# Cognoscan/entropy_coders

Measured on AMD Instinct MI355X. Metric: FSE encode+decode GiB/s on 1 GiB synthetic bytes; bit-exact round-trip, higher is better.
Workload: dtype u8

## Files before the change

entropy_coders_amd/csrc/fse_capi.cpp:

```cpp
#include <hip/hip_runtime.h>
#include <stdio.h>
#include <stdlib.h>
#include <string.h>

#include <algorithm>
#include <atomic>
#include <memory>
#include <mutex>
#include <thread>
#include <vector>

#include "../../include/fsehip.h"
#include "fse_kernels.h"

namespace {

constexpr uint32_t kDefaultBlock = 65536;
constexpr uint32_t kMaxBlock = 1u << 28;

uint64_t round_up(uint64_t x, uint64_t a) { return (x + a - 1) / a * a; }

enum {
    SCRATCH_DT = 0,
    SCRATCH_DTINFO = 1,
// ... 222 lines not shown
    uint8_t* buf[2] = {};
    size_t cap[2] = {};
    ~PinnedStaging() { release(); }
    void release() {
        for (int i = 0; i < 2; ++i) {
            if (buf[i]) (void)hipHostFree(buf[i]);
            buf[i] = nullptr;
            cap[i] = 0;
        }
    }
    uint8_t* get(int i, size_t bytes) {
        if (cap[i] < bytes) {
            if (buf[i]) (void)hipHostFree(buf[i]);
            buf[i] = nullptr;
            cap[i] = 0;
            void* p = nullptr;
            const size_t want = round_up(std::max<size_t>(bytes, size_t(64) << 10), 4096);
            if (hipHostMalloc(&p, want, hipHostMallocDefault) != hipSuccess) return nullptr;
            buf[i] = static_cast<uint8_t*>(p);
            cap[i] = want;
        }
        return buf[i];
    }
};
thread_local PinnedStaging g_pin;

struct Meta {
    uint32_t comp_len;
    uint32_t payload_bits;
    int32_t status;
    uint32_t pad;
};

int compress_one(const uint8_t* src, size_t n, uint32_t table_log, uint8_t* dst, size_t dst_cap, size_t* dst_len,
                 uint64_t* payload_bits, uint32_t nstates = 2) {
    if (!dst_len) return FSE_ERR_BAD_ARG;
    if (n == 0) return FSE_ERR_EMPTY;
    if (n > kMaxBlock) return FSE_ERR_UNSUPPORTED;
    if (table_log > 15) table_log = 15;
    if (!device_ok()) return FSE_ERR_NO_DEVICE;
    fsehip_params p{(uint32_t)round_up(n, 16), table_log, 0, table_log ? std::max<uint32_t>(table_log, 11) : 11,
                    nstates};
    const uint64_t slot = fsehip_slot_bytes(p.block_size, p.max_table_log);
    const size_t in_bytes = round_up(n, 16);
    const size_t pin_out = std::min<size_t>(slot, kPinOut);
    uint8_t* d_src = g_stage.get(0, in_bytes + 16);
    uint8_t* d_out = g_stage.get(1, slot);
    uint8_t* d_meta = g_stage.get(2, sizeof(Meta));
    uint8_t* h_in = g_pin.get(0, in_bytes);
    uint8_t* h_ret = g_pin.get(1, 256 + pin_out);
    if (!d_src || !d_out || !d_meta || !h_in || !h_ret) return FSE_ERR_HIP;
    memcpy(h_in, src, n);
    auto fail = [](int rc) {
        (void)hipStreamSynchronize(nullptr);
        return rc;
    };
    if (hipMemcpyAsync(d_src, h_in, in_bytes, hipMemcpyHostToDevice, nullptr) != hipSuccess) return fail(FSE_ERR_HIP);
    Meta* m = reinterpret_cast<Meta*>(d_meta);
    int rc = fsehip_compress_blocks(&p, d_src, n, d_out, slot, &m->comp_len, &m->payload_bits, nullptr,
                                    &m->status, nullptr);
    if (rc) return fail(rc);
    if (fsehip::launch_host_return(d_meta, d_out, &m->comp_len, h_ret, h_ret + 256, (uint32_t)pin_out, nullptr) !=
        hipSuccess)
        return fail(FSE_ERR_HIP);
    if (hipStreamSynchronize(nullptr) != hipSuccess) return FSE_ERR_HIP;
    Meta h;
    memcpy(&h, h_ret, sizeof h);
    if (h.status != FSE_OK) return h.status;
    if (*dst_len > dst_cap || dst_cap - *dst_len < h.comp_len) return FSE_ERR_DST_TOO_SMALL;
    const size_t head = std::min<size_t>(h.comp_len, pin_out);
    memcpy(dst + *dst_len, h_ret + 256, head);
    if (h.comp_len > head &&
        hipMemcpy(dst + *dst_len + head, d_out + head, h.comp_len - head, hipMemcpyDeviceToHost) != hipSuccess)
        return FSE_ERR_HIP;
    *dst_len += h.comp_len;
    if (payload_bits) *payload_bits = h.payload_bits;
    return FSE_OK;
}

}

extern "C" {

uint64_t fsehip_slot_bytes(uint32_t block_size, uint32_t max_table_log) {
    const uint64_t L = max_table_log ? max_table_log : 12;
    const uint64_t payload = ((uint64_t)block_size * L + 2 * L + 1 + 7) / 8;
    return round_up(512 + payload + 16, 256);
}

uint32_t fsehip_sidecar_per_block(uint32_t block_size, uint32_t ckpt_interval) {
    if (ckpt_interval == 0) return 0;
    return block_size / 2u / ckpt_interval + 2u;
}

uint32_t fsehip_sidecar_per_block_ns(uint32_t block_size, uint32_t ckpt_interval, uint32_t nstates) {
    if (ckpt_interval == 0) return 0;
    return nstates == 1 ? block_size / ckpt_interval + 2u : block_size / 2u / ckpt_interval + 2u;
}

int fsehip_device_count(void) {
    int n = 0;
    if (hipGetDeviceCount(&n) != hipSuccess) return 0;
    return n;
}

#ifdef FSEHIP_DIAG
const char* fsehip_version(void) { return "fsehip 0.2 (gfx950, diagnostics build: environment knobs live)"; }
#else
const char* fsehip_version(void) { return "fsehip 0.2 (gfx950)"; }
#endif

int fsehip_release_workspace(int device, fsehip_stream_t stream) {
    const int rc = release_workspaces(device, stream, false);
    g_stage.release();
    g_pin.release();
    return rc;
}

static int compress_blocks_impl(const fsehip_params* p, const uint8_t* d_src, uint64_t n_total, uint8_t* d_out,
                                uint64_t slot_bytes, uint32_t* d_comp_len, uint32_t* d_payload_bits,
                                uint64_t* d_sidecar, int32_t* d_status, fsehip_stream_t stream, Lease* held) {
    if (!p || !d_src || !d_out || !d_comp_len || !d_status) return FSE_ERR_BAD_ARG;
    if (n_total == 0) return FSE_ERR_EMPTY;
    const uint32_t bs = p->block_size ? p->block_size : kDefaultBlock;
    if (bs > kMaxBlock) return FSE_ERR_UNSUPPORTED;
    const uint64_t n_blocks = (n_total + bs - 1) / bs;
    if (n_blocks > 1 && (bs & 15u)) return FSE_ERR_BAD_ARG;
    if (n_blocks > 0xFFFFFFFFull) return FSE_ERR_BAD_ARG;
    const uint32_t lmax = kern_lmax(lmax_for(p));
    if (slot_bytes & 15u) return FSE_ERR_BAD_ARG;
    const uint32_t ns = p->nstates == 1 ? 1u : 2u;
    if (p->nstates > 2) return FSE_ERR_BAD_ARG;
    if (p->ckpt_interval && (p->ckpt_interval < (ns == 1 ? 16u : 8u) || (p->ckpt_interval & (p->ckpt_interval - 1))))
        return FSE_ERR_BAD_ARG;
    if (!device_ok()) return FSE_ERR_NO_DEVICE;
    fsehip::EncParams P{};
    P.nstates = ns;
    P.src = d_src;
    P.n_total = n_total;
    P.block_size = bs;
    P.n_blocks = (uint32_t)n_blocks;
    P.table_log = p->table_log;
    P.ckpt_interval = d_sidecar ? p->ckpt_interval : 0;
    P.ckpt_per_block = fsehip_sidecar_per_block_ns(bs, P.ckpt_interval, ns);
    P.out = d_out;
    P.slot_bytes = slot_bytes;
    P.comp_len = d_comp_len;
    P.payload_bits = d_payload_bits;
    P.sidecar = P.ckpt_interval ? d_sidecar : nullptr;
    P.status = d_status;
    P.lanes = (ns == 2 && env_u32("FSEHIP_ENC_LANES", 64) == 32) ? 32 : 64;
    P.debug = env_u32("FSEHIP_DEBUG", 0);
    P.xlds = env_u32("FSEHIP_ENC_XLDS", 0);
    P.rank_inject = env_u32("FSEHIP_RANK_INJECT", 0);
    const size_t groups = (n_blocks * P.lanes + 63) / 64;
    P.stamps = g_stamps_enc.get(groups);
    std::unique_ptr<Lease> lease;
    if (fsehip::enc_gsym(lmax) && slot_bytes < fsehip::ENC_SPREAD_OFF + (1ull << lmax)) {
        if (!held) lease = std::make_unique<Lease>(stream);
        P.spread = static_cast<uint8_t*>((held ? held : lease.get())->get(SCRATCH_SPREAD, n_blocks << lmax));
        if (!P.spread) return FSE_ERR_HIP;
    }
    hipError_t e = fsehip::launch_encode(P, lmax, static_cast<hipStream_t>(stream));
    if (P.stamps) g_stamps_enc.report("encode", groups, static_cast<hipStream_t>(stream));
    return e == hipSuccess ? FSE_OK : FSE_ERR_HIP;
}

int fsehip_compress_blocks(const fsehip_params* p, const uint8_t* d_src, uint64_t n_total, uint8_t* d_out,
                           uint64_t slot_bytes, uint32_t* d_comp_len, uint32_t* d_payload_bits, uint64_t* d_sidecar,
                           int32_t* d_status, fsehip_stream_t stream) {
    return compress_blocks_impl(p, d_src, n_total, d_out, slot_bytes, d_comp_len, d_payload_bits, d_sidecar, d_status,
                                stream, nullptr);
}

uint64_t fsehip_stream_out_bytes(uint32_t src_len, uint32_t max_table_log) {
    const uint64_t L = max_table_log ? std::min<uint32_t>(max_table_log, 15u) : 12;
    return round_up(512 + ((uint64_t)src_len * L + 2 * L + 1 + 7) / 8, 16);
}

int fsehip_compress_streams(uint32_t nstates, uint32_t table_log, uint32_t max_table_log, const uint8_t* d_src,
                            const fsehip_stream_desc* d_desc, uint32_t n_streams, uint8_t* d_out,
                            uint32_t* d_comp_len, uint32_t* d_payload_bits, int32_t* d_status,
                            fsehip_stream_t stream) {
    if (n_streams == 0) return FSE_OK;
    if (nstates > 2 || !d_src || !d_desc || !d_out || !d_comp_len || !d_status ||
        (reinterpret_cast<uintptr_t>(d_src) & 15u) || (reinterpret_cast<uintptr_t>(d_out) & 15u))
        return FSE_ERR_BAD_ARG;
    if (n_streams > (1u << 24) || max_table_log > 15) return FSE_ERR_UNSUPPORTED;
    if (!device_ok()) return FSE_ERR_NO_DEVICE;
    if (table_log > 15) table_log = 15;
    if (table_log && table_log < 5) table_log = 5;
    const fsehip_params p{0, table_log, 0, max_table_log, nstates};
    const uint32_t lmax = kern_lmax(lmax_for(&p));
    fsehip::EncParams P{};
    P.nstates = nstates == 1 ? 1u : 2u;
    P.src = d_src;
    P.n_blocks = n_streams;
    P.table_log = table_log;
    P.out = d_out;
    P.comp_len = d_comp_len;
    P.payload_bits = d_payload_bits;
    P.status = d_status;
    P.lanes = 64;
    P.desc = d_desc;
    std::unique_ptr<Lease> lease;
    if (fsehip::enc_gsym(lmax)) {
        lease = std::make_unique<Lease>(stream);
        P.spread = static_cast<uint8_t*>(lease->get(SCRATCH_SPREAD, (uint64_t)n_streams << lmax));
        if (!P.spread) return FSE_ERR_HIP;
    }
    return fsehip::launch_encode(P, lmax, static_cast<hipStream_t>(stream)) == hipSuccess ? FSE_OK : FSE_ERR_HIP;
}

static void defer_symbols(Lease& lease, fsehip::DecParams& P, uint32_t lmax) {
    if (lmax > 11 || P.block_size < 2u || P.n_blocks >= (1u << 24) || !env_u32("FSEHIP_SERIAL_DEFER", 1)) return;
    P.bulk = static_cast<uint32_t*>(lease.get(SCRATCH_BULK, 8ull * P.n_blocks, true));
    P.states = P.bulk ? static_cast<uint32_t*>(lease.get(SCRATCH_STATES, 2ull * P.n_blocks * P.block_size, true))
                      : nullptr;
    if (!P.states || !P.bulk) P.states = P.bulk = nullptr;
}

static int decompress_impl(const fsehip_params* p, const uint8_t* d_in, uint64_t slot_bytes,
                           const uint32_t* d_comp_len, const uint64_t* d_sidecar, uint8_t* d_out, uint64_t n_total,
                           uint64_t* d_sidecar_out, int32_t* d_status, uint32_t* d_out_len, uint32_t out_cap,
                           fsehip_stream_t stream, const uint32_t* d_dt, const int32_t* d_dtinfo,
                           Lease* lease = nullptr) {
    if (!p || !d_in || !d_comp_len || !d_out || !d_status || !d_dt || !d_dtinfo) return FSE_ERR_BAD_ARG;
    const uint32_t bs = p->block_size ? p->block_size : kDefaultBlock;
    if (bs > kMaxBlock) return FSE_ERR_UNSUPPORTED;
    const uint64_t n_blocks = n_total ? (n_total + bs - 1) / bs : 1;
    if (n_blocks > 1 && (bs & 15u)) return FSE_ERR_BAD_ARG;
    if (n_blocks > 0xFFFFFFFFull) return FSE_ERR_BAD_ARG;
    if ((slot_bytes & 31u) || (reinterpret_cast<uintptr_t>(d_in) & 15u) || (reinterpret_cast<uintptr_t>(d_out) & 15u))
        return FSE_ERR_BAD_ARG;
    const uint32_t ns = p->nstates == 1 ? 1u : 2u;
    if (p->nstates > 2) return FSE_ERR_BAD_ARG;
    if ((d_sidecar || d_sidecar_out) &&
        (p->ckpt_interval < (ns == 1 ? 16u : 8u) || (p->ckpt_interval & (p->ckpt_interval - 1))))
        return FSE_ERR_BAD_ARG;
    if (ns == 1 && d_sidecar_out && kern_lmax(p->max_table_log) > 12) return FSE_ERR_UNSUPPORTED;
    if (!device_ok()) return FSE_ERR_NO_DEVICE;
    fsehip::DecParams P{};
    P.nstates = ns;
    P.in = d_in;
    P.slot_bytes = slot_bytes;
    P.comp_len = d_comp_len;
    P.sidecar = d_sidecar;
    P.ckpt_interval = p->ckpt_interval;
    P.ckpt_per_block = fsehip_sidecar_per_block_ns(bs, p->ckpt_interval, ns);
    P.out = d_out;
    P.n_total = n_total;
    P.block_size = bs;
    P.n_blocks = (uint32_t)n_blocks;
    P.out_cap = out_cap;
    P.status = d_status;
    P.out_len = d_out_len;
    P.sidecar_out = d_sidecar_out;
    P.dt = d_dt;
    P.dtinfo = d_dtinfo;
    if (lease && !d_sidecar && !d_sidecar_out) defer_symbols(*lease, P, kern_lmax(p->max_table_log));
    P.stamps = g_stamps_dec.get(n_blocks);
    hipError_t e = fsehip::launch_decode(P, kern_lmax(p->max_table_log), static_cast<hipStream_t>(stream));
    if (P.stamps) g_stamps_dec.report("decode", n_blocks, static_cast<hipStream_t>(stream));
    return e == hipSuccess ? FSE_OK : FSE_ERR_HIP;
}

uint64_t fsehip_dtable_bytes(uint32_t max_table_log) { return 4ull << kern_lmax(max_table_log); }

static int build_dtables_impl(const fsehip_params* p, const uint8_t* d_in, uint64_t slot_bytes,
                              const uint32_t* d_comp_len, uint32_t n_blocks, uint32_t* d_dtables, int32_t* d_dtinfo,
                              fsehip_stream_t stream, Lease* lease) {
    if (!p || !d_in || !d_comp_len || !d_dtables || !d_dtinfo || (slot_bytes & 255u)) return FSE_ERR_BAD_ARG;
    if (n_blocks == 0) return FSE_OK;
    if (!device_ok()) return FSE_ERR_NO_DEVICE;
    fsehip::DtParams D{};
    if (lease && n_blocks >= 256u && kern_lmax(p->max_table_log) <= 12 && !env_u32("FSEHIP_DT_WAVE_PARSE", 0)) {
        uint8_t* h = static_cast<uint8_t*>(lease->get(SCRATCH_HDR, fsehip::hdr_scratch_bytes(n_blocks), true));
        if (h) {
            D.hdr_norm = reinterpret_cast<uint32_t*>(h);
            D.hdr_meta = reinterpret_cast<int2*>(h + 512ull * n_blocks);
        }
    }
    D.in = d_in;
    D.slot_bytes = slot_bytes;
    D.comp_len = d_comp_len;
    D.n_blocks = n_blocks;
    D.dt = d_dtables;
    D.dtinfo = d_dtinfo;
    D.xlds = env_u32("FSEHIP_DT_XLDS", 0);
    D.rank_inject = env_u32("FSEHIP_RANK_INJECT", 0);
    D.stamps = g_stamps_dt.get(n_blocks);
    hipError_t e = fsehip::launch_dtables(D, kern_lmax(p->max_table_log), static_cast<hipStream_t>(stream));
    if (D.stamps) g_stamps_dt.report("dtables", n_blocks, static_cast<hipStream_t>(stream));
    return e == hipSuccess ? FSE_OK : FSE_ERR_HIP;
}

int fsehip_build_dtables(const fsehip_params* p, const uint8_t* d_in, uint64_t slot_bytes, const uint32_t* d_comp_len,
                         uint32_t n_blocks, uint32_t* d_dtables, int32_t* d_dtinfo, fsehip_stream_t stream) {
    if (n_blocks < 256u) return build_dtables_impl(p, d_in, slot_bytes, d_comp_len, n_blocks, d_dtables, d_dtinfo, stream,
                                                   nullptr);
    Lease lease(stream);
    return build_dtables_impl(p, d_in, slot_bytes, d_comp_len, n_blocks, d_dtables, d_dtinfo, stream, &lease);
}

int fsehip_decompress_blocks_dt(const fsehip_params* p, const uint8_t* d_in, uint64_t slot_bytes,
                                const uint32_t* d_comp_len, const uint64_t* d_sidecar, const uint32_t* d_dtables,
                                const int32_t* d_dtinfo, uint8_t* d_out, uint64_t n_total, int32_t* d_status,
                                fsehip_stream_t stream) {
    if (n_total == 0) return FSE_ERR_EMPTY;
    if (!p || !d_dtables || !d_dtinfo) return FSE_ERR_BAD_ARG;
    if (d_sidecar && p->ckpt_interval == 0) return FSE_ERR_BAD_ARG;
    if (d_sidecar)
        return decompress_impl(p, d_in, slot_bytes, d_comp_len, d_sidecar, d_out, n_total, nullptr, d_status, nullptr,
                               0, stream, d_dtables, d_dtinfo);
    Lease lease(stream);
    return decompress_impl(p, d_in, slot_bytes, d_comp_len, nullptr, d_out, n_total, nullptr, d_status, nullptr, 0,
                           stream, d_dtables, d_dtinfo, &lease);
}

extern "C++" {
template <class Run>
static int with_dtables_lease(const fsehip_params* p, const uint8_t* d_in, uint64_t slot_bytes,
                              const uint32_t* d_comp_len, uint64_t n_blocks, fsehip_stream_t stream, Lease& lease,
                              Run run) {
    uint32_t* dt = static_cast<uint32_t*>(lease.get(SCRATCH_DT, fsehip_dtable_bytes(p->max_table_log) * n_blocks));
    int32_t* info = static_cast<int32_t*>(lease.get(SCRATCH_DTINFO, 4ull * n_blocks));
    if (!dt || !info) return FSE_ERR_HIP;
    int rc = build_dtables_impl(p, d_in, slot_bytes, d_comp_len, (uint32_t)n_blocks, dt, info, stream, &lease);
    return rc != FSE_OK ? rc : run(dt, info, lease);
}
template <class Run>
static int with_dtables_n(const fsehip_params* p, const uint8_t* d_in, uint64_t slot_bytes, const uint32_t* d_comp_len,
                          uint64_t n_blocks, fsehip_stream_t stream, Run run) {
    if (n_blocks > 0xFFFFFFFFull) return FSE_ERR_BAD_ARG;
    if (!device_ok()) return FSE_ERR_NO_DEVICE;
    Lease lease(stream);
    return with_dtables_lease(p, d_in, slot_bytes, d_comp_len, n_blocks, stream, lease, run);
}
template <class Run>
static int with_dtables(const fsehip_params* p, const uint8_t* d_in, uint64_t slot_bytes, const uint32_t* d_comp_len,
                        uint64_t n_total, fsehip_stream_t stream, Run run) {
    const uint32_t bs = p->block_size ? p->block_size : kDefaultBlock;
    if (bs > kMaxBlock) return FSE_ERR_UNSUPPORTED;
    return with_dtables_n(p, d_in, slot_bytes, d_comp_len, (n_total + bs - 1) / bs, stream, run);
}
}

int fsehip_decompress_blocks(const fsehip_params* p, const uint8_t* d_in, uint64_t slot_bytes,
                             const uint32_t* d_comp_len, const uint64_t* d_sidecar, uint8_t* d_out, uint64_t n_total,
                             int32_t* d_status, fsehip_stream_t stream) {
    if (n_total == 0) return FSE_ERR_EMPTY;
    if (!p) return FSE_ERR_BAD_ARG;
    if (d_sidecar && p->ckpt_interval == 0) return FSE_ERR_BAD_ARG;
    return with_dtables(p, d_in, slot_bytes, d_comp_len, n_total, stream,
                        [&](const uint32_t* dt, const int32_t* info, Lease& lease) {
                            return decompress_impl(p, d_in, slot_bytes, d_comp_len, d_sidecar, d_out, n_total, nullptr,
// ... 1043 lines not shown
```

entropy_coders_amd/csrc/fse_kernels.h:

```cpp
#pragma once
#include <hip/hip_runtime.h>
#include <stdint.h>

#include "../../include/fsehip.h"

namespace fsehip {

struct EncParams {
    const uint8_t* src;
    uint64_t n_total;
    uint32_t block_size;
    uint32_t n_blocks;
    uint32_t table_log;
    uint32_t ckpt_interval;
    uint32_t ckpt_per_block;
    uint8_t* out;
    uint64_t slot_bytes;
    uint32_t* comp_len;
    uint32_t* payload_bits;
    uint64_t* sidecar;
    int32_t* status;
    uint32_t lanes;
    uint32_t nstates;
    uint32_t debug;
    uint64_t* stamps;
    uint32_t xlds;
    uint32_t peer_ranks;
    uint32_t rank_inject;
    uint8_t* spread;
    const fsehip_stream_desc* desc;
};
constexpr bool enc_gsym(uint32_t lmax) { return lmax >= 13u; }
constexpr uint32_t ENC_SPREAD_OFF = 512;

struct DecParams {
    const uint8_t* in;
    uint64_t slot_bytes;
    const uint32_t* comp_len;
    const uint64_t* sidecar;
    uint32_t ckpt_interval;
    uint32_t ckpt_per_block;
    uint8_t* out;
    uint64_t n_total;
    uint32_t block_size;
    uint32_t n_blocks;
    uint32_t out_cap;
    int32_t* status;
    uint32_t* out_len;
    uint64_t* sidecar_out;
    uint64_t* stamps;
    const uint32_t* dt;
    const int32_t* dtinfo;
    uint32_t pass;
    uint32_t nstates;
    uint32_t* states;
    uint32_t* bulk;
};

struct DtParams {
    const uint8_t* in;
    uint64_t slot_bytes;
    const uint32_t* comp_len;
    uint32_t n_blocks;
    uint32_t* dt;
    int32_t* dtinfo;
    uint32_t xlds;
    uint64_t* stamps;
    int2* hdr_meta;
    uint32_t* hdr_norm;
    uint32_t peer_ranks;
    uint32_t rank_inject;
};
constexpr uint64_t hdr_scratch_bytes(uint64_t n_blocks) { return n_blocks * (512u + 8u); }

struct GenParams {
    uint8_t* out;
    uint64_t n_total;
    uint64_t block_size;
    uint64_t seed;
    int32_t kind;
    uint32_t nsym;
    uint16_t bound[1024];
};

struct NormArgs {
    int mode;
    const uint8_t* src;
    uint64_t n;
    const uint32_t* counts;
    uint32_t size, table_len, log2;
    fse_norm_histogram* out;
    uint32_t* counts_out;
    int32_t* status;
};
hipError_t launch_norm(const NormArgs& A, hipStream_t s);
hipError_t launch_hdr_write(const fse_norm_histogram* nh, uint8_t* out, uint32_t* bits, int32_t* status, hipStream_t s);
hipError_t launch_hdr_read(const uint8_t* src, uint32_t n, fse_norm_histogram* out, uint32_t* used, int32_t* status,
                           hipStream_t s);
hipError_t launch_table(const fse_norm_histogram* nh, int enc, fse_encode_table* et, fse_decode_table* dt,
                        int32_t* status, hipStream_t s);
hipError_t rank_order_check(uint32_t* violations, uint64_t* atomics);
hipError_t rank_fallbacks_enc(uint32_t* out, bool reset);
hipError_t rank_fallbacks_dec(uint32_t* out, bool reset);
hipError_t rank_fallbacks_tab(uint32_t* out, bool reset);
bool atomic_ranks_on();
int rank_mode(int mode);
hipError_t launch_host_return(const void* meta, const uint8_t* src, const uint32_t* len, void* hmeta, uint8_t* hdst,
                              uint32_t max, hipStream_t s);
uint64_t bits_tiles(uint64_t count);
hipError_t launch_bits_scan(const uint8_t* nbits, const uint8_t* ops, uint64_t count, uint32_t* tile_sum,
                            uint64_t* tile_off, uint64_t* total, hipStream_t s);
hipError_t launch_bits_pack(const uint32_t* vals, const uint8_t* nbits, uint64_t count, const uint64_t* tile_off,
                            const uint64_t* total, uint32_t* out, uint64_t lim_words, hipStream_t s);
hipError_t launch_bits_unpack(const uint8_t* in, uint64_t n_bytes, uint64_t total_bits, int stack,
                              const uint8_t* nbits, const uint8_t* ops, uint64_t count, const uint64_t* tile_off,
                              const uint64_t* total, uint32_t* vals, uint64_t* result, hipStream_t s);

#ifndef FSEHIP_KSTAMPS
#define FSEHIP_KSTAMPS
constexpr int kStamps = 10;
#endif
constexpr int32_t FSE_DEFERRED = 1;

hipError_t launch_encode(const EncParams& P, uint32_t lmax, hipStream_t stream);
hipError_t launch_dtables(const DtParams& P, uint32_t lmax, hipStream_t stream);
hipError_t launch_decode(const DecParams& P, uint32_t lmax, hipStream_t stream);
hipError_t launch_single(const DecParams& P, uint32_t lmax, hipStream_t stream);
constexpr uint32_t single_ftab_bytes() { return 2048u * 8u; }
int occupancy_report(char* buf, int cap);
int occupancy_report_dec(char* buf, int cap);
hipError_t launch_histogram(const uint8_t* src, uint64_t n_total, uint32_t block_size, uint32_t n_blocks,
                            uint32_t* counts, uint32_t* table_len, hipStream_t stream);
hipError_t launch_generate(const GenParams& G, hipStream_t stream);
hipError_t launch_pack(const uint8_t* slots, uint64_t slot_bytes, const uint32_t* comp_len, const uint64_t* offsets,
                       uint32_t n_blocks, uint8_t* stream, int unpack, hipStream_t hs);
hipError_t launch_copy(const uint8_t* src, const uint64_t* src_off, const uint32_t* lens, uint32_t n_blocks,
                       uint8_t* dst, const uint64_t* dst_off, hipStream_t hs);

hipError_t launch_stream_offsets(const uint32_t* lens, uint32_t n, uint64_t* offsets, uint64_t* total,
                                 hipStream_t hs);

struct FrameHdr {
    uint32_t w[8];
};
struct FrameChunk {
    uint8_t* frame;
    uint64_t frame_len;
    uint64_t n_total;
    uint32_t block_size, ckpt_interval, nstates, n_blocks;
    uint32_t c0, cb;
    uint8_t* slots;
    uint64_t slot_bytes;
    uint32_t* comp_len;
    int32_t* status;
    uint64_t* sidecar;
    uint32_t spb;
    uint32_t* kind;
    uint64_t* off;
    uint64_t* base;
    uint8_t* raw;
};
hipError_t launch_frame_plan(const FrameChunk& F, const FrameHdr& hdr, bool first, bool last, uint64_t* frame_len,
                             int32_t* result, hipStream_t hs);
hipError_t launch_frame_pack(const FrameChunk& F, hipStream_t hs);
hipError_t launch_frame_check(const FrameChunk& F, const FrameHdr& hdr, int32_t* result, hipStream_t hs);
hipError_t launch_frame_scan(const FrameChunk& F, hipStream_t hs);
hipError_t launch_frame_unpack(const FrameChunk& F, hipStream_t hs);
hipError_t launch_frame_merge(const FrameChunk& F, int32_t* block_status, int32_t* result, hipStream_t hs);

}
```

entropy_coders_amd/csrc/fse_kernels.hip:

```cpp

#include "fse_device.hpp"
#include "fse_kernels.h"

namespace fsehip {

__device__ uint32_t g_rank_fb_enc;
hipError_t rank_fallbacks_enc(uint32_t* out, bool reset) {
    hipError_t e = hipMemcpyFromSymbol(out, HIP_SYMBOL(g_rank_fb_enc), 4, 0, hipMemcpyDeviceToHost);
    if (e == hipSuccess && reset) {
        const uint32_t z = 0;
        e = hipMemcpyToSymbol(HIP_SYMBOL(g_rank_fb_enc), &z, 4, 0, hipMemcpyHostToDevice);
    }
    return e;
}


__device__ __forceinline__ uint4 load_chunk(const uint8_t* blk, uint32_t n, uint32_t c) {
    const uint32_t off = c << 4;
    if (off + 16u <= n) return *reinterpret_cast<const uint4*>(blk + off);
    uint32_t w[4] = {0, 0, 0, 0};
    for (uint32_t i = 0; i < 16u && off + i < n; ++i) w[i >> 2] |= (uint32_t)blk[off + i] << (8u * (i & 3u));
    return make_uint4(w[0], w[1], w[2], w[3]);
}

// ... 283 lines not shown
}
template <int NS>
__device__ __forceinline__ void ckpt_record(Ckpt& ck, uint32_t p, uint32_t pos, uint32_t x0, uint32_t x1) {
    const uint64_t e = ckpt_entry<NS>(ck, pos, x0, x1);
    if (ck.queue) {
#pragma unroll
        for (int i = (int)CKQ - 1; i > 0; --i) ck.q[i] = ck.q[i - 1];
        ck.q[0] = e;
        ck.lo = p >> ck.shift;
        ++ck.cnt;
    } else {
        ck.base[p >> ck.shift] = e;
    }
}
__device__ __forceinline__ void ckpt_flush(const Ckpt& ck) {
    if (!ck.queue) return;
#pragma unroll
    for (uint32_t i = 0; i < CKQ; ++i)
        if (i < ck.cnt) ck.base[ck.lo + i] = ck.q[i];
}

template <int MODE, int NS>
__device__ __forceinline__ EncState enc_range(const uint8_t* __restrict__ blk, uint32_t n, uint32_t pa, uint32_t pb,
                                              EncState st, const EncTab& T, Emit& em, Ckpt& ck, Track& tr) {
    constexpr bool TRACK = counts<MODE>();
    constexpr bool RP = MODE == PASS_REPAIR;
    uint32_t x0 = st.x0, x1 = st.x1, b0 = st.b0, b1 = st.b1;
    if (pb <= pa) return st;
    const uint4* v = reinterpret_cast<const uint4*>(blk);
    constexpr uint32_t CS = NS == 2 ? 3u : 4u;
    int32_t c_hi = (int32_t)((pb - 1u) >> CS);
    const int32_t c_lo = (int32_t)(pa >> CS);
    uint32_t rem = 0, slot = 0;
    if (TRACK) {
        rem = (uint32_t)(c_hi - c_lo) % tr.ckc;
        slot = (uint32_t)(c_hi - c_lo) / tr.ckc;
    }
    auto track = [&]() {
        if (rem == 0u) {
            const uint32_t sv = x0 | (x1 << 16);
            if (RP) {
                if (tr.cx[slot] == sv) {
                    const uint2 r = tr.cb[slot];
                    tr.done = true;
                    tr.jstar = slot;
                    b0 += r.x;
                    b1 += r.y;
                } else {
                    tr.cx[slot] = sv;
                    tr.cb[slot] = make_uint2(b0, b1);
                }
            } else {
                tr.cx[slot] = sv;
                tr.cb[slot] = make_uint2(b0, b1);
            }
            slot -= 1u;
            rem = tr.ckc - 1u;
        } else {
            rem -= 1u;
        }
    };
    if (pb & ((1u << CS) - 1u)) {
        const uint4 q = load_chunk(blk, n, (uint32_t)c_hi);
        enc_chunk<MODE, false, NS>(q, (uint32_t)c_hi << CS, pb, x0, x1, T, b0, b1, em);
        if (emits<MODE>()) em.drain();
        if (MODE == PASS_EMIT && ck.base && (((uint32_t)c_hi << CS) & ck.mask) == 0u)
            ckpt_record<NS>(ck, (uint32_t)c_hi << CS, em.pos(), x0, x1);
        if (TRACK) track();
        c_hi -= 1;
    }
    if (c_hi < c_lo || (RP && tr.done)) return EncState{x0, x1, b0, b1};
    auto ld = [&](int32_t c) { return v[c < c_lo ? c_lo : c]; };
    constexpr int PF = ENC_PF;
    uint4 q[PF];
#pragma unroll
    for (int k = 0; k < PF; ++k) q[k] = ld(c_hi - k);
    uint2 t0[8], t1[8];
    tt_load(q[0], t0, t1, T);
    auto body = [&](const uint4& q, const uint4& qn, int32_t c) {
        (void)q;
        enc_chunk_pl<MODE, NS>(qn, t0, t1, x0, x1, T, b0, b1, em);
        if (emits<MODE>()) em.drain();
        if (MODE == PASS_EMIT && ck.base && (((uint32_t)c << CS) & ck.mask) == 0u)
            ckpt_record<NS>(ck, (uint32_t)c << CS, em.pos(), x0, x1);
        if (TRACK) track();
    };
    auto stop = [&](int32_t cn) { return cn < c_lo || (RP && tr.done); };
    for (int32_t c = c_hi;; c -= PF) {
        bool done = false;
#pragma unroll
        for (int k = 0; k < PF; ++k) {
            body(q[k], q[(k + 1) % PF], c - k);
            if (stop(c - k - 1)) {
                done = true;
                break;
            }
            q[k] = ld(c - k - PF);
        }
        if (done) break;
    }
    return EncState{x0, x1, b0, b1};
}

__device__ __forceinline__ uint32_t enc_init(const EncTab& T, uint32_t s) {
    const uint2 t = T.tt[s];
    const uint32_t bo = (t.x + (1u << 15)) >> 16;
    const uint32_t v = (bo << 16) - t.x;
    return st_at(((v >> bo) << 1) + t.y);
}

template <int MODE, int NS>
__device__ __forceinline__ EncState top_start(const uint8_t* blk, uint32_t n, const EncTab& tab, Emit& em) {
    EncState e;
    e.b0 = e.b1 = 0;
    if (NS == 1) {
        e.x0 = enc_init(tab, blk[n - 1u]);
        e.x1 = 0;
        return e;
    }
    if (n & 1u) {
        e.x0 = enc_init(tab, blk[n - 1u]);
        e.x1 = enc_init(tab, blk[n - 2u]);
        const uint32_t v0 = e.x0;
        const uint32_t nb = enc_step(e.x0, blk[n - 3u], tab);
        if (MODE == PASS_COUNT) e.b0 = nb;
        if (MODE == PASS_EMIT) {
            em.put(v0 & ((1u << nb) - 1u), nb);
            em.flush();
        }
    } else {
        e.x0 = enc_init(tab, blk[n - 2u]);
        e.x1 = enc_init(tab, blk[n - 1u]);
    }
    return e;
}

template <int BPW>
struct EncTail {
    int32_t status[BPW];
    uint32_t L[BPW];
    uint32_t hl[BPW];
    uint32_t hv[BPW];
    int scratch[4];
};

template <int LMAX, int T>
struct EncSmem {
    static constexpr int BPW = 64 / T;
    static constexpr uint32_t SIZE = 1u << LMAX;
    static constexpr bool TAIL_IN_P2 = LMAX >= 14;
    static_assert(!TAIL_IN_P2 || BPW == 1, "one block per wave");
    static constexpr uint32_t HS = BPW == 1 ? HSUB : 8u;
    static_assert(BPW == 1 || 2u * SIZE >= hist_words<8>() * 4u, "sub-histograms fit the stateTable");
    union {
        struct {
            __attribute__((aligned(16))) uint16_t st[BPW][SIZE];
            uint2 tt[BPW][256];
        };
        __attribute__((aligned(16))) uint32_t hist[BPW == 1 ? hist_words<HS>() : 4];
    };
    union {
        struct {
            union {
                uint32_t hdrw[HDR_MAX / 4];
                __attribute__((aligned(16))) uint8_t sym_at[enc_gsym(LMAX) ? 16u : SIZE];
            } u;
            int32_t norm[256];
            uint16_t cumul[256];
            uint32_t cnt[256];
        } p1;
        union {
            struct {
                uint2 cb[64 * track_slots<LMAX>()];
                uint32_t cx[64 * track_slots<LMAX>()];
                uint32_t cntF[BPW][T + 1];
                EncTail<BPW> tail[TAIL_IN_P2 ? 1 : 0];
            } u;
            __attribute__((aligned(16))) uint32_t ring[64 * RING_STRIDE];
            struct {
                uint32_t mword[BPW][2 * (T + 1)];
                uint32_t mval[BPW][2 * (T + 1)];
            } mg;
        } p2;
    } ph;
    EncTail<BPW> tail_out[TAIL_IN_P2 ? 0 : 1];
    __device__ __forceinline__ EncTail<BPW>& tail() {
        if constexpr (TAIL_IN_P2) return ph.p2.u.tail[0];
        else return tail_out[0];
    }
};

struct EncGeom {
    const uint8_t* blk;
    uint32_t n;
    uint8_t* out;
    uint64_t cap;
    int pre;
};
template <bool STREAMS>
__device__ __forceinline__ EncGeom enc_geom(const EncParams& P, uint64_t gb) {
    if constexpr (STREAMS) {
        const fsehip_stream_desc d = P.desc[gb];
        const int pre = ((d.src_off | d.out_off) & 15u) ? FSE_ERR_BAD_ARG
                        : d.src_len > (1u << 28)        ? FSE_ERR_UNSUPPORTED
                                                        : FSE_OK;
        return EncGeom{P.src + d.src_off, pre == FSE_OK ? d.src_len : 0u, P.out + d.out_off, d.out_cap, pre};
    } else {
        const uint64_t off = gb * P.block_size;
        return EncGeom{P.src + off, (uint32_t)min((uint64_t)P.block_size, P.n_total - off), P.out + gb * P.slot_bytes,
                       P.slot_bytes, FSE_OK};
    }
}

template <int LMAX, int T, int NS, bool STREAMS>
__device__ __forceinline__ void encode_body(const EncParams& P, EncSmem<LMAX, T>& sm) {
    constexpr int BPW = 64 / T;
    static_assert(!EncSmem<LMAX, T>::TAIL_IN_P2 ||
                      64u * track_slots<LMAX>() * 12u + 4u * (T + 1u) >= sizeof(sm.ph.p1),
                  "tail overlaps phase-1 scratch");
#define ENC_WGID ((uint64_t)blockIdx.x)
#define ENC_SYNC() __syncthreads()
    const uint32_t lane = lane_id();

    FSE_STAMP(P, 0);
    for (int b = 0; b < BPW; ++b) {
        const uint64_t gb = ENC_WGID * BPW + b;
        if (gb >= P.n_blocks) {
            if (lane == 0) sm.tail().status[b] = 1;
            continue;
        }
        const EncGeom G = enc_geom<STREAMS>(P, gb);
        const uint32_t n = G.n;
        const uint8_t* blk = G.blk;
        uint32_t* counts = sm.ph.p1.cnt;
        using Sm = EncSmem<LMAX, T>;
        const uint32_t tl = wave_histogram<Sm::HS>(
            blk, n, BPW == 1 ? sm.hist : reinterpret_cast<uint32_t*>(sm.st[b]), counts);
        FSE_STAMP(P, 1);
        if (FSE_ABLATE(P, 8u)) {
            if (lane == 0) P.status[gb] = (int32_t)tl;
            continue;
        }
        int rc = G.pre;
        uint32_t Lreq = P.table_log, L = 0, slow = 0;
        if (rc == FSE_OK && n == 0) rc = FSE_ERR_EMPTY;
        if (rc == FSE_OK && P.table_log == 0) rc = optimal_log2(n, tl, &Lreq);
        if (rc == FSE_OK) rc = wave_normalize(counts, n, tl, Lreq, sm.ph.p1.norm, &L, &slow, sm.tail().scratch);
        if (rc == FSE_OK && n < 2) rc = FSE_ERR_TOO_SHORT;
        if (rc == FSE_OK && L > (uint32_t)LMAX) rc = FSE_ERR_UNSUPPORTED;
        FSE_STAMP(P, 2);
        if (rc == FSE_OK) {
            const int hl = wave_header_write(sm.ph.p1.norm, L, tl, sm.ph.p1.u.hdrw);
            if (lane == 0) sm.tail().scratch[1] = hl;
            if (hl < 0) {
                rc = hl;
            } else {
                const uint32_t* h = sm.ph.p1.u.hdrw;
                uint32_t* gw = reinterpret_cast<uint32_t*>(G.out);
                if (!STREAMS || (uint64_t)hl <= G.cap)
                    for (uint32_t w = lane; w < (uint32_t)hl / 4u; w += WAVE) gw[w] = h[w];
                if (lane == 0) sm.tail().hv[b] = (hl & 3) ? h[hl / 4] & ((1u << (8u * (hl & 3))) - 1u) : 0u;
            }
            wave_sync();
        }
        FSE_STAMP(P, 3);
        if (rc == FSE_OK) {
            const uint32_t size = 1u << L;
            uint16_t* st = sm.st[b];
            const uint16_t* cumul = sm.ph.p1.cumul;
            constexpr bool GSYM = enc_gsym(LMAX);
            uint8_t* const sym_at = !GSYM ? sm.ph.p1.u.sym_at
                                    : (STREAMS || P.spread) ? P.spread + gb * (uint64_t)(1u << LMAX)
                                                            : G.out + ENC_SPREAD_OFF;
            static_assert(ENC_SPREAD_OFF >= HDR_MAX && ENC_SPREAD_OFF % 16u == 0u, "in-slot spread array");
            rc = wave_build_spread<64, false, GSYM>(sm.ph.p1.norm, L, tl, sym_at, reinterpret_cast<uint8_t*>(st), sm.ph.p1.cumul,
                                   sm.ph.p1.cnt,
                                   [&](uint32_t i, uint32_t, uint32_t r) {
                                       st[r] = (uint16_t)(size + i);
                                   },
                                   [&](uint32_t s) { return (uint32_t)cumul[s]; },
                                   RankAtomic{P.peer_ranks == 0u, nullptr, st, size, &g_rank_fb_enc, P.rank_inject}, nullptr,
                                   reinterpret_cast<uint64_t*>(&sm.tt[b][0]));
            const uint32_t stb = lds_addr_of(&sm.st[b][0]);
            for (uint32_t s = lane; s < 256; s += WAVE) {
                int32_t x = (s < tl) ? sm.ph.p1.norm[s] : 0;
                uint2 t = make_uint2(0, stb);
                if (s < tl) {
                    const int32_t tot = (int32_t)sm.ph.p1.cumul[s];
                    if (x == 0) {
                        t.x = ((L + 1u) << 16) - (1u << L);
                    } else if (x == -1 || x == 1) {
                        t.x = (L << 16) - (1u << L);
                        t.y = stb + (uint32_t)(2 * (tot - 1));
                    } else {
                        const uint32_t mb = L - ilog2u((uint32_t)(x - 1));
                        t.x = (mb << 16) - ((uint32_t)x << mb);
                        t.y = stb + (uint32_t)(2 * (tot - x));
                    }
                }
                sm.tt[b][s] = t;
            }
            wave_sync();
            if (lane == 0) {
                auto init_ok = [&](uint32_t s) {
                    const uint2 t = sm.tt[b][s];
                    const uint32_t bo = (t.x + (1u << 15)) >> 16;
                    const uint32_t v = (bo << 16) - t.x;
                    const int32_t idx = (int32_t)((v >> bo) + (uint32_t)((int32_t)(t.y - stb) >> 1));
                    return idx >= 0 && idx < (int32_t)size;
                };
                const bool ok = init_ok(blk[n - 1u]) && (NS == 1 || init_ok(blk[n - 2u]));
                sm.tail().scratch[2] = ok ? FSE_OK : FSE_ERR_ENCODER_INIT;
            }
            wave_sync();
            if (rc == FSE_OK) rc = sm.tail().scratch[2];
        }
        if (lane == 0) {
            const uint32_t hl = (rc == FSE_OK) ? (uint32_t)sm.tail().scratch[1] : 0u;
            sm.tail().status[b] = rc;
            sm.tail().L[b] = L;
            sm.tail().hl[b] = hl;
            if (rc != FSE_OK) {
                P.status[gb] = rc;
                P.comp_len[gb] = 0;
                if (P.payload_bits) P.payload_bits[gb] = 0;
            }
        }
        ENC_SYNC();
    }

    FSE_STAMP(P, 4);
    if (FSE_ABLATE(P, 9u)) return;
    const int b = BPW == 1 ? 0 : (int)(lane / T);
    const uint32_t k = BPW == 1 ? lane : lane % T;
    const uint64_t gb = ENC_WGID * BPW + b;
    const bool live = sm.tail().status[b] == FSE_OK;
    using Sm2 = EncSmem<LMAX, T>;
    const uint32_t hl_early = Sm2::TAIL_IN_P2 ? sm.tail().hl[b] : 0u;
    const uint32_t hv_early = Sm2::TAIL_IN_P2 ? sm.tail().hv[b] : 0u;
    const EncGeom G = live ? enc_geom<STREAMS>(P, gb) : EncGeom{P.src, 0u, P.out, 0u, FSE_OK};
    const uint32_t n = G.n;
    const uint8_t* blk = G.blk;
    const uint32_t L = sm.tail().L[b];
    const EncTab tab{sm.tt[b]};
    const uint32_t Pm = live ? (NS == 2 ? ((n & 1u) ? (n - 3u) / 2u : n / 2u - 1u) : n - 1u) : 0u;
    constexpr uint32_t SPC = NS == 2 ? 8u : 16u;
    uint32_t S = (Pm + T - 1u) / T;
    S = max(SPC, (S + SPC - 1u) & ~(SPC - 1u));
    const uint32_t ktop = Pm ? (Pm - 1u) / S : 0u;
    const bool act = live && k <= ktop;
    const uint32_t pa = k * S, pb = min(pa + S, Pm);
    Emit em;
    em.start(nullptr, 0);
    Ckpt ck{nullptr, 0, 0, 0, L, false, 0, 0, {}};

    constexpr uint32_t TS = track_slots<LMAX>();
    Track tr{&sm.ph.p2.u.cx[lane * TS], &sm.ph.p2.u.cb[lane * TS], max(1u, (S / SPC + TS - 1u) / TS), false, 0u};
    const uint32_t nslot = pb > pa ? (((pb - 1u) / SPC) - (pa / SPC)) / tr.ckc + 1u : 0u;
    uint32_t start = (1u << L) | (NS == 2 ? (1u << L) << 16 : 0u);
    uint32_t bits = 0;
    uint32_t tot0 = 0, tot1 = 0;
    uint32_t myF = 0;
    uint32_t n_iter = 0, n_rerun = 0;
    {
        constexpr int MC = PASS_COUNT, MR = PASS_REPAIR;
        if (act) {
            EncState e0 = (k == ktop) ? top_start<PASS_COUNT, NS>(blk, n, tab, em)
                                      : EncState{start & 0xFFFFu, start >> 16, 0u, 0u};
            e0 = enc_range<MC, NS>(blk, n, pa, pb, e0, tab, em, ck, tr);
            tot0 = e0.b0;
            tot1 = e0.b1;
            myF = e0.x0 | (e0.x1 << 16);
            sm.ph.p2.u.cntF[b][k] = myF;
            track_fixup(tr, nslot, -1, tot0, tot1);
        }
        FSE_STAMP(P, 5);
        for (;;) {
            if (FSE_ABLATE(P, 16u)) break;
            ENC_SYNC();
            bool bad0 = false, bad1 = false;
            uint32_t nbF = 0;
            if (act && k < ktop) {
                nbF = sm.ph.p2.u.cntF[b][k + 1];
                bad0 = ((nbF ^ start) & 0xFFFFu) != 0u;
                bad1 = ((nbF ^ start) >> 16) != 0u;
            }
            const bool bad = bad0 || bad1;
            ENC_SYNC();
            if (__ballot(bad) == 0) break;
            ++n_iter;
// ... 138 lines not shown
#undef ENC_WGID

template <int LMAX, int T, int NS>
__global__ __launch_bounds__(64) void encode_blocks_kernel(EncParams P) {
    __shared__ EncSmem<LMAX, T> sm;
    encode_body<LMAX, T, NS, false>(P, sm);
}
template <int LMAX, int T, int NS>
__global__ __launch_bounds__(64) void encode_streams_kernel(EncParams P) {
    __shared__ EncSmem<LMAX, T> sm;
    encode_body<LMAX, T, NS, true>(P, sm);
}

__global__ __launch_bounds__(64) void histogram_blocks_kernel(const uint8_t* src, uint64_t n_total,
                                                              uint32_t block_size, uint32_t n_blocks,
                                                              uint32_t* counts, uint32_t* table_len) {
    __shared__ uint32_t h4[HIST_WORDS];
    __shared__ uint32_t cnts[256];
    const uint64_t gb = blockIdx.x;
    if (gb >= n_blocks) return;
    const uint64_t off = gb * block_size;
    const uint32_t n = (uint32_t)min((uint64_t)block_size, n_total - off);
    const uint32_t tl = wave_histogram(src + off, n, h4, cnts);
    for (uint32_t s = lane_id(); s < 256; s += WAVE) counts[gb * 256 + s] = cnts[s];
    if (lane_id() == 0 && table_len) table_len[gb] = tl;
}

__global__ __launch_bounds__(256) void pack_blocks_kernel(const uint8_t* __restrict__ slots, uint64_t slot_bytes,
                                                          const uint32_t* __restrict__ comp_len,
                                                          const uint64_t* __restrict__ offsets, uint32_t n_blocks,
                                                          uint8_t* __restrict__ stream, int unpack) {
    const uint64_t b = blockIdx.x;
    if (b >= n_blocks) return;
    const uint32_t len = comp_len[b];
    uint8_t* slot = const_cast<uint8_t*>(slots) + b * slot_bytes;
    const uint64_t o = offsets[b];
    if (!unpack) {
        const uint64_t d0 = (o + 3u) >> 2, d1 = (o + len) >> 2;
        const uint32_t* src = reinterpret_cast<const uint32_t*>(slot);
        uint32_t* dst = reinterpret_cast<uint32_t*>(stream);
        if (d1 > d0) {
            const uint32_t head = (uint32_t)(4u * d0 - o);
            for (uint64_t d = d0 + threadIdx.x; d < d1; d += 256u) {
                const uint32_t sb = head + 4u * (uint32_t)(d - d0);
                const uint32_t q = sb >> 2, sh = sb & 3u;
                const uint32_t lo = src[q], hi = sh ? src[q + 1u] : 0u;
                dst[d] = __builtin_amdgcn_alignbyte(hi, lo, sh);
            }
        }
        const uint64_t hb = min((uint64_t)len, 4u * d0 - o);
        if (threadIdx.x < hb) stream[o + threadIdx.x] = slot[threadIdx.x];
        const uint64_t tb0 = d1 > d0 ? 4u * d1 - o : hb;
        for (uint64_t i = tb0 + threadIdx.x; i < len; i += 256u) stream[o + i] = slot[i];
    } else {
        const uint8_t* s = stream + o;
        for (uint32_t i = threadIdx.x; i < len; i += 256u) slot[i] = s[i];
    }
}

__global__ __launch_bounds__(256) void copy_blocks_kernel(const uint8_t* __restrict__ src,
                                                          const uint64_t* __restrict__ src_off,
                                                          const uint32_t* __restrict__ lens, uint32_t n_blocks,
                                                          uint8_t* __restrict__ dst,
                                                          const uint64_t* __restrict__ dst_off) {
    const uint64_t b = blockIdx.x;
    if (b >= n_blocks) return;
    const uint32_t len = lens[b];
    const uint64_t so = src_off[b], o = dst_off[b];
    const uint64_t d0 = (o + 3u) >> 2, d1 = (o + len) >> 2;
    uint32_t* dw = reinterpret_cast<uint32_t*>(dst);
    if (d1 > d0) {
        const uint64_t s0 = so + (4u * d0 - o);
        const uint32_t sh = (uint32_t)(s0 & 3u);
        const uint32_t* sw = reinterpret_cast<const uint32_t*>(src) + (s0 >> 2);
        for (uint64_t d = threadIdx.x; d < d1 - d0; d += 256u) {
            const uint32_t lo = sw[d];
            const uint32_t hi = sh ? sw[d + 1u] : 0u;
            dw[d0 + d] = __builtin_amdgcn_alignbyte(hi, lo, sh);
        }
    }
    const uint64_t hb = min((uint64_t)len, 4u * d0 - o);
    if (threadIdx.x < hb) dst[o + threadIdx.x] = src[so + threadIdx.x];
    const uint64_t tb0 = d1 > d0 ? 4u * d1 - o : hb;
    for (uint64_t i = tb0 + threadIdx.x; i < len; i += 256u) dst[o + i] = src[so + i];
}

__global__ __launch_bounds__(1024) void stream_offsets_kernel(const uint32_t* __restrict__ lens, uint32_t n,
                                                              uint64_t* __restrict__ offsets,
                                                              uint64_t* __restrict__ total) {
    __shared__ uint64_t part[1024];
    const uint32_t t = threadIdx.x;
    const uint32_t per = (n + 1023u) / 1024u;
    const uint32_t lo = (uint32_t)min((uint64_t)t * per, (uint64_t)n), hi = (uint32_t)min((uint64_t)lo + per, (uint64_t)n);
    auto r16 = [](uint32_t x) { return ((uint64_t)x + 15u) & ~15ull; };
    uint64_t s = 0;
    for (uint32_t i = lo; i < hi; ++i) s += r16(lens[i]);
    part[t] = s;
    __syncthreads();
    for (uint32_t d = 1; d < 1024u; d <<= 1) {
        const uint64_t v = t >= d ? part[t - d] : 0ull;
        __syncthreads();
        part[t] += v;
        __syncthreads();
    }
    uint64_t o = part[t] - s;
    for (uint32_t i = lo; i < hi; ++i) {
        offsets[i] = o;
        o += r16(lens[i]);
    }
    if (t == 1023u) *total = part[1023];
}

__device__ __forceinline__ uint64_t mix64(uint64_t z) {
    z = (z ^ (z >> 30)) * 0xBF58476D1CE4E5B9ull;
    z = (z ^ (z >> 27)) * 0x94D049BB133111EBull;
    return z ^ (z >> 31);
}

__global__ __launch_bounds__(256) void generate_kernel(GenParams G) {
    const uint64_t GOLDEN = 0x9E3779B97F4A7C15ull;
    const uint64_t i16 = ((uint64_t)blockIdx.x * blockDim.x + threadIdx.x) * 16ull;
    if (i16 >= G.n_total) return;
    uint32_t w[4] = {0, 0, 0, 0};
    for (int j = 0; j < 16; ++j) {
        const uint64_t i = i16 + j;
        if (i >= G.n_total) break;
        const uint64_t b = i / G.block_size, r = i - b * G.block_size;
        const uint64_t sb = G.seed ^ (b * GOLDEN);
        const uint64_t x = mix64(sb + (r + 1ull) * GOLDEN);
        uint32_t v;
        if (G.kind == 0) {
            const uint32_t idx = (uint32_t)(x & 4095u);
            uint32_t lo = 0, hi = G.nsym - 1u;
            while (lo < hi) {
                const uint32_t mid = (lo + hi + 1u) >> 1;
                if (G.bound[mid] <= idx) lo = mid; else hi = mid - 1u;
            }
            v = lo & 0xFFu;
        } else if (G.kind == 1) {
            const uint32_t c = (uint32_t)__builtin_ctzll(x | (1ull << 63));
            v = c > 255u ? 255u : c;
        } else {
            v = (uint32_t)(((x >> 32) * 240ull) >> 32);
        }
        w[j >> 2] |= v << (8 * (j & 3));
    }
    if (i16 + 16 <= G.n_total) {
        *reinterpret_cast<uint4*>(G.out + i16) = make_uint4(w[0], w[1], w[2], w[3]);
    } else {
        for (uint64_t j = 0; i16 + j < G.n_total; ++j) G.out[i16 + j] = (uint8_t)(w[j >> 2] >> (8 * (j & 3)));
    }
}

constexpr uint32_t ENC_WGS = 11u;
hipError_t launch_encode(const EncParams& P0, uint32_t lmax, hipStream_t stream) {
    EncParams P = P0;
    P.peer_ranks = atomic_ranks_on() ? 0u : 1u;
    const uint32_t T = (P.lanes == 32 && lmax <= 12) ? 32u : 64u;
    const uint32_t bpw = 64u / T;
    const dim3 g((P.n_blocks + bpw - 1u) / bpw), b(64);
    auto go = [&](auto kern, uint32_t pad = 0) { hipLaunchKernelGGL(kern, g, b, P.xlds ? P.xlds : pad, stream, P); };
    if (P.desc) {
        if (enc_gsym(lmax) && !P.spread) return hipErrorInvalidValue;
        const dim3 gs(P.n_blocks);
        auto gos = [&](auto kern, uint32_t pad = 0) { hipLaunchKernelGGL(kern, gs, b, pad, stream, P); };
        if (P.nstates == 1) {
            if (lmax <= 11) gos(encode_streams_kernel<11, 64, 1>);
            else if (lmax <= 12) gos(encode_streams_kernel<12, 64, 1>);
            else if (lmax <= 13) gos(encode_streams_kernel<13, 64, 1>);
            else if (lmax <= 14) gos(encode_streams_kernel<14, 64, 1>);
            else gos(encode_streams_kernel<15, 64, 1>);
        } else {
            static const uint32_t pad11s = [] {
                hipFuncAttributes fa{};
                if (hipFuncGetAttributes(&fa, reinterpret_cast<const void*>(encode_streams_kernel<11, 64, 2>)) !=
                    hipSuccess)
                    return 0u;
                const size_t per = (160u << 10) / ENC_WGS - 64u;
                return fa.sharedSizeBytes < per ? (uint32_t)(per - fa.sharedSizeBytes) : 0u;
            }();
            if (lmax <= 11) gos(encode_streams_kernel<11, 64, 2>, pad11s);
            else if (lmax <= 12) gos(encode_streams_kernel<12, 64, 2>);
            else if (lmax <= 13) gos(encode_streams_kernel<13, 64, 2>);
            else if (lmax <= 14) gos(encode_streams_kernel<14, 64, 2>);
            else gos(encode_streams_kernel<15, 64, 2>);
        }
        return hipGetLastError();
    }
    if (P.nstates == 1) {
        if (lmax <= 11) go(encode_blocks_kernel<11, 64, 1>);
        else if (lmax <= 12) go(encode_blocks_kernel<12, 64, 1>);
        else if (lmax <= 13) go(encode_blocks_kernel<13, 64, 1>);
        else if (lmax <= 14) go(encode_blocks_kernel<14, 64, 1>);
        else go(encode_blocks_kernel<15, 64, 1>);
    } else if (T == 64) {
        static const uint32_t pad11 = [] {
            hipFuncAttributes fa{};
            if (hipFuncGetAttributes(&fa, reinterpret_cast<const void*>(encode_blocks_kernel<11, 64, 2>)) != hipSuccess)
                return 0u;
            const size_t per = (160u << 10) / ENC_WGS - 64u;
            return fa.sharedSizeBytes < per ? (uint32_t)(per - fa.sharedSizeBytes) : 0u;
        }();
        if (lmax <= 11) go(encode_blocks_kernel<11, 64, 2>, pad11);
        else if (lmax <= 12) go(encode_blocks_kernel<12, 64, 2>);
        else if (lmax <= 13) go(encode_blocks_kernel<13, 64, 2>);
        else if (lmax <= 14) go(encode_blocks_kernel<14, 64, 2>);
        else go(encode_blocks_kernel<15, 64, 2>);
    } else {
        if (lmax <= 11) go(encode_blocks_kernel<11, 32, 2>);
        else go(encode_blocks_kernel<12, 32, 2>);
    }
    return hipGetLastError();
}

int occupancy_report(char* buf, int cap) {
    int len = 0;
    auto one = [&](const char* name, const void* k, int threads) {
        int nb = -1;
        hipFuncAttributes fa{};
        (void)hipOccupancyMaxActiveBlocksPerMultiprocessor(&nb, k, threads, 0);
        (void)hipFuncGetAttributes(&fa, k);
        if (len < cap)
            len += snprintf(buf + len, cap - len, "%s: %d WG/CU (lds %zu B, vgpr %d)\n", name, nb,
                            fa.sharedSizeBytes, fa.numRegs);
    };
    one("encode<11,64,2>", reinterpret_cast<const void*>(encode_blocks_kernel<11, 64, 2>), 64);
    one("encode<15,64,2>", reinterpret_cast<const void*>(encode_blocks_kernel<15, 64, 2>), 64);
    return len;
}

hipError_t launch_histogram(const uint8_t* src, uint64_t n_total, uint32_t block_size, uint32_t n_blocks,
                            uint32_t* counts, uint32_t* table_len, hipStream_t stream) {
    hipLaunchKernelGGL(histogram_blocks_kernel, dim3(n_blocks), dim3(64), 0, stream, src, n_total, block_size,
                       n_blocks, counts, table_len);
    return hipGetLastError();
}

hipError_t launch_pack(const uint8_t* slots, uint64_t slot_bytes, const uint32_t* comp_len, const uint64_t* offsets,
                       uint32_t n_blocks, uint8_t* stream, int unpack, hipStream_t hs) {
    hipLaunchKernelGGL(pack_blocks_kernel, dim3(n_blocks), dim3(256), 0, hs, slots, slot_bytes, comp_len, offsets,
                       n_blocks, stream, unpack);
    return hipGetLastError();
}

hipError_t launch_copy(const uint8_t* src, const uint64_t* src_off, const uint32_t* lens, uint32_t n_blocks,
                       uint8_t* dst, const uint64_t* dst_off, hipStream_t hs) {
    hipLaunchKernelGGL(copy_blocks_kernel, dim3(n_blocks), dim3(256), 0, hs, src, src_off, lens, n_blocks, dst,
                       dst_off);
    return hipGetLastError();
}

hipError_t launch_stream_offsets(const uint32_t* lens, uint32_t n, uint64_t* offsets, uint64_t* total,
                                 hipStream_t hs) {
    hipLaunchKernelGGL(stream_offsets_kernel, dim3(1), dim3(1024), 0, hs, lens, n, offsets, total);
    return hipGetLastError();
}

hipError_t launch_generate(const GenParams& G, hipStream_t stream) {
    const uint64_t threads = (G.n_total + 15) / 16;
    const uint32_t grid = (uint32_t)((threads + 255) / 256);
    hipLaunchKernelGGL(generate_kernel, dim3(grid), dim3(256), 0, stream, G);
    return hipGetLastError();
}

}
```

Before: 501.5.

## Overlay encoder sub-histograms on live LDS and drop forced LDS padding

For one-block-per-wave encoders with LMAX<=11, the sub-histogram scratch now aliases the start of the shared-memory struct instead of sitting in a separate union member. A static_assert guards that this overlay does not clobber phase-1 counters or the tail. The default LDS padding that capped residency at 11 workgroups per CU is removed (ENC_WGS=0). Padding is now computed only when an FSEHIP_ENC_WGS env override is set, rounded to the LDS allocation granule. Together these shrink per-workgroup LDS and let the hardware pick occupancy, at the cost of possibly more cache or LDS contention.

```diff
diff --git a/entropy_coders_amd/csrc/fse_capi.cpp b/entropy_coders_amd/csrc/fse_capi.cpp
--- a/entropy_coders_amd/csrc/fse_capi.cpp
+++ b/entropy_coders_amd/csrc/fse_capi.cpp
@@ -398,6 +398,7 @@
     P.lanes = (ns == 2 && env_u32("FSEHIP_ENC_LANES", 64) == 32) ? 32 : 64;
     P.debug = env_u32("FSEHIP_DEBUG", 0);
     P.xlds = env_u32("FSEHIP_ENC_XLDS", 0);
+    P.enc_wgs = env_u32("FSEHIP_ENC_WGS", 0);
     P.rank_inject = env_u32("FSEHIP_RANK_INJECT", 0);
     const size_t groups = (n_blocks * P.lanes + 63) / 64;
     P.stamps = g_stamps_enc.get(groups);
@@ -448,6 +449,7 @@
     P.payload_bits = d_payload_bits;
     P.status = d_status;
     P.lanes = 64;
+    P.enc_wgs = env_u32("FSEHIP_ENC_WGS", 0);
     P.desc = d_desc;
     std::unique_ptr<Lease> lease;
     if (fsehip::enc_gsym(lmax)) {
diff --git a/entropy_coders_amd/csrc/fse_kernels.h b/entropy_coders_amd/csrc/fse_kernels.h
--- a/entropy_coders_amd/csrc/fse_kernels.h
+++ b/entropy_coders_amd/csrc/fse_kernels.h
@@ -27,6 +27,7 @@
     uint32_t xlds;
     uint32_t peer_ranks;
     uint32_t rank_inject;
+    uint32_t enc_wgs;
     uint8_t* spread;
     const fsehip_stream_desc* desc;
 };
diff --git a/entropy_coders_amd/csrc/fse_kernels.hip b/entropy_coders_amd/csrc/fse_kernels.hip
--- a/entropy_coders_amd/csrc/fse_kernels.hip
+++ b/entropy_coders_amd/csrc/fse_kernels.hip
@@ -459,12 +459,14 @@
     static_assert(!TAIL_IN_P2 || BPW == 1, "one block per wave");
     static constexpr uint32_t HS = BPW == 1 ? HSUB : 8u;
     static_assert(BPW == 1 || 2u * SIZE >= hist_words<8>() * 4u, "sub-histograms fit the stateTable");
+    static constexpr bool HIST_OVERLAY = BPW == 1 && LMAX <= 11;
+    static constexpr uint32_t HIST_BYTES = hist_words<HS>() * 4u;
     union {
         struct {
             __attribute__((aligned(16))) uint16_t st[BPW][SIZE];
             uint2 tt[BPW][256];
         };
-        __attribute__((aligned(16))) uint32_t hist[BPW == 1 ? hist_words<HS>() : 4];
+        __attribute__((aligned(16))) uint32_t hist[BPW == 1 && !HIST_OVERLAY ? hist_words<HS>() : 4];
     };
     union {
         struct {
@@ -495,7 +497,20 @@
         if constexpr (TAIL_IN_P2) return ph.p2.u.tail[0];
         else return tail_out[0];
     }
+    __device__ __forceinline__ uint32_t* hist_view() {
+        if constexpr (HIST_OVERLAY) return reinterpret_cast<uint32_t*>(this);
+        else return hist;
+    }
 };
+template <int LMAX, int T>
+constexpr bool enc_overlay_ok() {
+    using S = EncSmem<LMAX, T>;
+    if (!S::HIST_OVERLAY) return sizeof(S::hist) >= (S::BPW == 1 ? S::HIST_BYTES : 16u);
+    return offsetof(S, st) == 0 && S::HIST_BYTES > offsetof(S, ph) &&
+           offsetof(S, ph) + offsetof(decltype(S::ph), p1.cumul) >= S::HIST_BYTES &&
+           offsetof(S, ph) + offsetof(decltype(S::ph), p1.cnt) >= S::HIST_BYTES &&
+           offsetof(S, tail_out) >= S::HIST_BYTES && !S::TAIL_IN_P2;
+}
 
 struct EncGeom {
     const uint8_t* blk;
@@ -525,6 +540,7 @@
     static_assert(!EncSmem<LMAX, T>::TAIL_IN_P2 ||
                       64u * track_slots<LMAX>() * 12u + 4u * (T + 1u) >= sizeof(sm.ph.p1),
                   "tail overlaps phase-1 scratch");
+    static_assert(enc_overlay_ok<LMAX, T>(), "sub-histogram view over live phase-1 bytes");
 #define ENC_WGID ((uint64_t)blockIdx.x)
 #define ENC_SYNC() __syncthreads()
     const uint32_t lane = lane_id();
@@ -542,7 +558,7 @@
         uint32_t* counts = sm.ph.p1.cnt;
         using Sm = EncSmem<LMAX, T>;
         const uint32_t tl = wave_histogram<Sm::HS>(
-            blk, n, BPW == 1 ? sm.hist : reinterpret_cast<uint32_t*>(sm.st[b]), counts);
+            blk, n, BPW == 1 ? sm.hist_view() : reinterpret_cast<uint32_t*>(sm.st[b]), counts);
         FSE_STAMP(P, 1);
         if (FSE_ABLATE(P, 8u)) {
             if (lane == 0) P.status[gb] = (int32_t)tl;
@@ -987,7 +1003,23 @@
     }
 }
 
-constexpr uint32_t ENC_WGS = 11u;
+constexpr uint32_t LDS_GRANULE = 1280u, LDS_CU = 160u << 10;
+constexpr uint32_t ENC_WGS = 0u;
+template <auto KERN>
+uint32_t enc_static_lds() {
+    static const uint32_t lds = [] {
+        hipFuncAttributes fa{};
+        return hipFuncGetAttributes(&fa, reinterpret_cast<const void*>(KERN)) == hipSuccess ? (uint32_t)fa.sharedSizeBytes
+                                                                                             : 0u;
+    }();
+    return lds;
+}
+template <auto KERN>
+uint32_t enc_pad(uint32_t wgs) {
+    if (wgs == 0u) return 0u;
+    const uint32_t lds = enc_static_lds<KERN>(), per = LDS_CU / wgs / LDS_GRANULE * LDS_GRANULE;
+    return lds && lds < per ? per - lds : 0u;
+}
 hipError_t launch_encode(const EncParams& P0, uint32_t lmax, hipStream_t stream) {
     EncParams P = P0;
     P.peer_ranks = atomic_ranks_on() ? 0u : 1u;
@@ -995,26 +1027,19 @@
     const uint32_t bpw = 64u / T;
     const dim3 g((P.n_blocks + bpw - 1u) / bpw), b(64);
     auto go = [&](auto kern, uint32_t pad = 0) { hipLaunchKernelGGL(kern, g, b, P.xlds ? P.xlds : pad, stream, P); };
+    const uint32_t wgs = P.enc_wgs ? P.enc_wgs : ENC_WGS;
     if (P.desc) {
         if (enc_gsym(lmax) && !P.spread) return hipErrorInvalidValue;
         const dim3 gs(P.n_blocks);
         auto gos = [&](auto kern, uint32_t pad = 0) { hipLaunchKernelGGL(kern, gs, b, pad, stream, P); };
         if (P.nstates == 1) {
-            if (lmax <= 11) gos(encode_streams_kernel<11, 64, 1>);
+            if (lmax <= 11) gos(encode_streams_kernel<11, 64, 1>, enc_pad<encode_streams_kernel<11, 64, 1>>(wgs));
             else if (lmax <= 12) gos(encode_streams_kernel<12, 64, 1>);
             else if (lmax <= 13) gos(encode_streams_kernel<13, 64, 1>);
             else if (lmax <= 14) gos(encode_streams_kernel<14, 64, 1>);
             else gos(encode_streams_kernel<15, 64, 1>);
         } else {
-            static const uint32_t pad11s = [] {
-                hipFuncAttributes fa{};
-                if (hipFuncGetAttributes(&fa, reinterpret_cast<const void*>(encode_streams_kernel<11, 64, 2>)) !=
-                    hipSuccess)
-                    return 0u;
-                const size_t per = (160u << 10) / ENC_WGS - 64u;
-                return fa.sharedSizeBytes < per ? (uint32_t)(per - fa.sharedSizeBytes) : 0u;
-            }();
-            if (lmax <= 11) gos(encode_streams_kernel<11, 64, 2>, pad11s);
+            if (lmax <= 11) gos(encode_streams_kernel<11, 64, 2>, enc_pad<encode_streams_kernel<11, 64, 2>>(wgs));
             else if (lmax <= 12) gos(encode_streams_kernel<12, 64, 2>);
             else if (lmax <= 13) gos(encode_streams_kernel<13, 64, 2>);
             else if (lmax <= 14) gos(encode_streams_kernel<14, 64, 2>);
@@ -1023,20 +1048,13 @@
         return hipGetLastError();
     }
     if (P.nstates == 1) {
-        if (lmax <= 11) go(encode_blocks_kernel<11, 64, 1>);
+        if (lmax <= 11) go(encode_blocks_kernel<11, 64, 1>, enc_pad<encode_blocks_kernel<11, 64, 1>>(wgs));
         else if (lmax <= 12) go(encode_blocks_kernel<12, 64, 1>);
         else if (lmax <= 13) go(encode_blocks_kernel<13, 64, 1>);
         else if (lmax <= 14) go(encode_blocks_kernel<14, 64, 1>);
         else go(encode_blocks_kernel<15, 64, 1>);
     } else if (T == 64) {
-        static const uint32_t pad11 = [] {
-            hipFuncAttributes fa{};
-            if (hipFuncGetAttributes(&fa, reinterpret_cast<const void*>(encode_blocks_kernel<11, 64, 2>)) != hipSuccess)
-                return 0u;
-            const size_t per = (160u << 10) / ENC_WGS - 64u;
-            return fa.sharedSizeBytes < per ? (uint32_t)(per - fa.sharedSizeBytes) : 0u;
-        }();
-        if (lmax <= 11) go(encode_blocks_kernel<11, 64, 2>, pad11);
+        if (lmax <= 11) go(encode_blocks_kernel<11, 64, 2>, enc_pad<encode_blocks_kernel<11, 64, 2>>(wgs));
         else if (lmax <= 12) go(encode_blocks_kernel<12, 64, 2>);
         else if (lmax <= 13) go(encode_blocks_kernel<13, 64, 2>);
         else if (lmax <= 14) go(encode_blocks_kernel<14, 64, 2>);
```

New measurement: 514.0, median of 6. 1.02x the previous value.
